# yhhshb/biolib

Hardware: AMD Instinct MI355X
Metric: Gbp/s minimizer-scanned (k=31,w=11) (higher is better)
Workload: dtype u64

## Files before the change

biolib_amd/csrc/bl_capi.hip:

```cpp
#include <hip/hip_runtime.h>
#include <algorithm>
#include <cstdio>
#include <cstdlib>
#include <cstring>
#include <deque>
#include <new>
#include <string>
#include <utility>
#include <vector>

#include "../../include/biolib_amd.h"
#include "bl_host.hpp"
#include "bl_launch.hpp"
#include "bl_lookup_launch.hpp"
#include "bl_read_counts_launch.hpp"
#include "bl_scan128_launch.hpp"

namespace {

thread_local std::string g_err;

int fail(int code, const std::string& msg)
{
    g_err = msg;
// ... 1 lines not shown
}

}

int bl_set_error(int code, const char* msg) { return fail(code, msg ? msg : ""); }

namespace {

#define BL_HIP(call)                                                                                       \
    do {                                                                                                   \
        hipError_t e_ = (call);                                                                            \
        if (e_ != hipSuccess)                                                                              \
            return fail(e_ == hipErrorOutOfMemory ? BL_ERR_OOM : BL_ERR_HIP,                               \
                        std::string(#call) + ": " + hipGetErrorString(e_));                                \
    } while (0)

constexpr int RESULT_WORDS = 16;
constexpr int RING = 256;
constexpr size_t HDR_BYTES = 256;
constexpr size_t SHARD_BYTES = (size_t)bl::NSHARD * 8 * sizeof(unsigned long long);

struct Pending {
    bl_result* user;
    int slot;
    uint64_t capacity;
    bool has_capacity;
};

}

struct Lane {
    hipStream_t own = nullptr;
    unsigned char* ws = nullptr;
    size_t ws_bytes = 0;
    unsigned char* tile_buf = nullptr;
    size_t tile_buf_bytes = 0;
    uint16_t* slot_buf = nullptr;
    size_t slot_buf_bytes = 0;
    hipEvent_t ev_start = nullptr, ev_stop = nullptr;
    hipEvent_t ev_count_done = nullptr;
    bool count_recorded = false;
    bool scan_recorded = false;

    unsigned long long* shards() const { return reinterpret_cast<unsigned long long*>(ws + HDR_BYTES); }
    unsigned long long* result() const { return reinterpret_cast<unsigned long long*>(ws + HDR_BYTES + SHARD_BYTES); }
};

struct bl_ctx {
    int device = 0;
    Lane lanes[2];
    Lane* cur = nullptr;
    int next_lane = 0;
    int n_lanes = 1;
    uint32_t emit_lds_per_wg = 0;
    hipStream_t user_stream = nullptr;
    bool borrowed = false;
    hipStream_t stream = nullptr;
    unsigned long long* pinned = nullptr;
    hipEvent_t slot_ev[RING] = {};
    int next_slot = 0;
    std::deque<Pending> pending;
    bool timed = false;
    bool exact_windows = false;
    bool position_tiled = false;
    bool packed_codes = true;
    bool direct_codes = true;
    int jaccard128_path = 0;
    bool count128_tables = true;
    int table_prefix_bits = -1;
    bool ktiming = false;
    bl::LaunchLog last_kernels{};
    std::vector<hipEvent_t> ev_pool;
    std::vector<std::pair<hipEvent_t, hipEvent_t>> ev_open;
    double kernel_ms = 0.0;
    uint64_t kernel_launches = 0;
    std::vector<std::pair<hipEvent_t, hipEvent_t>> marks;
    std::vector<bl_batch*> batches;
    void* scratch[8] = {};
    size_t scratch_bytes[8] = {};
    std::vector<std::pair<void*, size_t>> pool_idle;
    std::vector<std::pair<void*, size_t>> pool_live;

    unsigned long long* shards() const { return cur->shards(); }
    unsigned long long* result() const { return cur->result(); }
    static size_t fixed_bytes() { return HDR_BYTES + SHARD_BYTES + RESULT_WORDS * sizeof(unsigned long long); }
};

struct bl_batch {
    bl_ctx* ctx = nullptr;
    uint8_t* bases = nullptr;
    bool owns_bases = false;
    uint32_t* start_bits = nullptr;
    uint32_t* packed = nullptr;
    uint32_t* codes = nullptr;
    uint32_t* chunk_bad = nullptr;
    uint64_t n_bases = 0;
    uint64_t n_seqs = 0;
    uint64_t read_len = 0;
    uint64_t origin = 0;
};

namespace {

int grow(bl_ctx* c, void** buf, size_t* have, size_t need)
{
    if (need <= *have) return BL_OK;
    BL_HIP(hipStreamSynchronize(c->stream));
    if (*buf) BL_HIP(hipFree(*buf));
    *buf = nullptr;
    *have = 0;
    const size_t bytes = need + need / 8;
    hipError_t e = hipMalloc(buf, bytes);
    if (e != hipSuccess) return fail(BL_ERR_OOM, std::string("hipMalloc(scan scratch): ") + hipGetErrorString(e));
    *have = bytes;
    return BL_OK;
}

int ensure_workspace(bl_ctx* c)
{
    return grow(c, reinterpret_cast<void**>(&c->cur->ws), &c->cur->ws_bytes, bl_ctx::fixed_bytes());
}

void select_lane(bl_ctx* c)
{
    if (c->borrowed) {
        c->cur = &c->lanes[0];
        c->stream = c->user_stream;
    } else {
        c->cur = &c->lanes[c->next_lane];
        if (c->n_lanes == 2) c->next_lane ^= 1;
        c->stream = c->cur->own;
    }
}

void deliver(bl_ctx* c, const Pending& p)
{
    const unsigned long long* r = c->pinned + (size_t)p.slot * RESULT_WORDS;
    bl_result out;
    std::memset(&out, 0, sizeof(out));
    out.count = r[0];
    out.xor_value = r[1];
    out.xor_hash = r[2];
    out.xor_pos = r[3];
    out.aux = r[4];
    out.redone = (int32_t)(r[5] > 0x7fffffffull ? 0x7fffffffull : r[5]);
    out.status = BL_OK;
    if (p.has_capacity && r[0] > p.capacity) out.status = BL_ERR_CAPACITY;
    if (p.user) *p.user = out;
}

int flush_pending(bl_ctx* c)
{
// ... 18 lines not shown

int sync_ctx(bl_ctx* c)
{
    for (Lane& l : c->lanes) BL_HIP(hipStreamSynchronize(l.own));
    if (c->borrowed) BL_HIP(hipStreamSynchronize(c->user_stream));
    int rc = flush_kernel_events(c);
    if (rc != BL_OK) return rc;
    return flush_pending(c);
}

int kernel_event(bl_ctx* c, bool start)
{
    if (!c->ktiming) return BL_OK;
    if (start) {
        hipEvent_t ev[2];
        for (int i = 0; i < 2; ++i) {
            if (!c->ev_pool.empty()) { ev[i] = c->ev_pool.back(); c->ev_pool.pop_back(); }
            else BL_HIP(hipEventCreate(&ev[i]));
        }
        c->ev_open.emplace_back(ev[0], ev[1]);
        BL_HIP(hipEventRecord(ev[0], c->stream));
    } else {
        BL_HIP(hipEventRecord(c->ev_open.back().second, c->stream));
    }
    return BL_OK;
}

int begin_scan(bl_ctx* c)
{
    BL_HIP(hipSetDevice(c->device));
    select_lane(c);
    int rc = ensure_workspace(c);
    if (rc != BL_OK) return rc;
    BL_HIP(hipEventRecord(c->cur->ev_start, c->stream));
    BL_HIP(hipMemsetAsync(c->cur->ws, 0, bl_ctx::fixed_bytes(), c->stream));
    return BL_OK;
}

int end_scan(bl_ctx* c, uint32_t add_mask, bl_result* user, bool has_capacity, uint64_t capacity, uint32_t flags,
             bool already_folded = false)
{
    if (!already_folded) {
        hipError_t e = bl::launch_reduce_shards(c->shards(), c->result(), add_mask, reinterpret_cast<unsigned long long*>(c->cur->ws) + 1, c->stream);
        if (e != hipSuccess) return fail(BL_ERR_HIP, std::string("reduce_shards: ") + hipGetErrorString(e));
    }
    if ((int)c->pending.size() >= RING) {
        const Pending old = c->pending.front();
        BL_HIP(hipEventSynchronize(c->slot_ev[old.slot]));
        deliver(c, old);
        c->pending.pop_front();
    }
    const int slot = c->next_slot;
    c->next_slot = (c->next_slot + 1) % RING;
    BL_HIP(hipMemcpyAsync(c->pinned + (size_t)slot * RESULT_WORDS, c->result(), RESULT_WORDS * sizeof(unsigned long long),
                          hipMemcpyDeviceToHost, c->stream));
    BL_HIP(hipEventRecord(c->slot_ev[slot], c->stream));
    BL_HIP(hipEventRecord(c->cur->ev_stop, c->stream));
    c->cur->scan_recorded = true;
    c->timed = true;
    c->pending.push_back(Pending{user, slot, capacity, has_capacity});
    if (flags & BL_FLAG_SYNC) {
        int rc = sync_ctx(c);
        if (rc != BL_OK) return rc;
        if (user && user->status != BL_OK)
            return fail(user->status, "output capacity too small for the records found");
    }
    return BL_OK;
}

int zero_result(bl_ctx* c, bl_result* user, uint32_t flags)
{
    if (user) std::memset(user, 0, sizeof(*user));
    (void)c;
    (void)flags;
    return BL_OK;
}

int check_range(const bl_batch* b, uint64_t first, uint64_t n, uint64_t& end)
{
    if (first > b->n_bases) return fail(BL_ERR_INVALID, "range starts beyond the batch");
    end = (n == 0 || n > b->n_bases - first) ? b->n_bases : first + n;
    if (end - first > (1ull << 31)) return fail(BL_ERR_INVALID, "a scan range may hold at most 2^31 positions; split it");
    return BL_OK;
}

int make_start_bits(bl_ctx* c, bl_batch* b, const uint64_t* offsets, uint64_t n_seqs, uint64_t read_len)
{
    const uint64_t n_words = (b->n_bases + 31) / 32 + 4;
    if (!offsets && (read_len == 0 || read_len >= b->n_bases)) {
        b->start_bits = nullptr;
// ... 29 lines not shown
    const uint64_t total = (uint64_t)bl::packed_total((int64_t)b->n_bases);
    b->packed = static_cast<uint32_t*>(bl_ctx_pool_alloc(c, (total + total / 32) * sizeof(uint32_t)));
    if (!b->packed) return fail(BL_ERR_OOM, "device allocation of the batch's packed codes failed (bl_ctx_set_option(\"packed_codes\", 0) does without)");
    b->codes = b->packed + bl::PACK_LEAD;
    b->chunk_bad = b->packed + total + bl::PACK_LEAD / 32;
    hipError_t e = bl::launch_pack_codes(b->bases, b->n_bases, b->packed, b->packed + total, s);
    if (e != hipSuccess) return fail(BL_ERR_HIP, std::string("pack_codes: ") + hipGetErrorString(e));
    return BL_OK;
}

int ensure_start_bits(bl_ctx* c, const bl_batch* cb)
{
    bl_batch* b = const_cast<bl_batch*>(cb);
    if (b->start_bits || b->read_len == 0 || b->read_len >= b->n_bases) return BL_OK;
    int rc = sync_ctx(c);
    if (rc != BL_OK) return rc;
    return make_start_bits(c, b, nullptr, 0, b->read_len);
}

}

int bl_ctx_kernel_event(bl_ctx* c, hipStream_t stream, int start)
{
    const hipStream_t keep = c->stream;
    c->stream = stream;
    const int rc = kernel_event(c, start != 0);
    c->stream = keep;
    return rc;
}

hipStream_t bl_ctx_stream(bl_ctx* c)
{
    if (c->borrowed) return c->user_stream;
    if (c->n_lanes == 2 && c->lanes[1].scan_recorded) (void)hipStreamWaitEvent(c->lanes[0].own, c->lanes[1].ev_stop, 0);
    return c->lanes[0].own;
}
int bl_ctx_device(bl_ctx* c) { return c->device; }
int bl_ctx_count128_tables(bl_ctx* c) { return c->count128_tables ? 1 : 0; }
int bl_ctx_jaccard128_path(bl_ctx* c) { return c->jaccard128_path; }
int bl_ctx_table_prefix_bits(bl_ctx* c) { return c->table_prefix_bits; }
int bl_batch_describe(const bl_batch* b, bl_ctx** ctx, uint64_t* n_bases, uint64_t* n_seqs, uint64_t* read_len)
{
    *ctx = b->ctx;
    *n_bases = b->n_bases;
    *n_seqs = b->n_seqs;
    *read_len = b->read_len;
    return BL_OK;
}

int bl_batch_scan_view(bl_ctx* c, const bl_batch* b, int ensure, const uint32_t** start_bits)
{
    if (ensure) {
        int rc = ensure_start_bits(c, b);
        if (rc != BL_OK) return rc;
    }
    *start_bits = b->start_bits;
    return BL_OK;
}

void* bl_ctx_scratch(bl_ctx* c, int slot, size_t bytes)
{
    if (!c || slot < 0 || slot >= 8) return nullptr;
    if (bytes <= c->scratch_bytes[slot]) return c->scratch[slot];
    (void)hipSetDevice(c->device);
    if (c->scratch[slot]) {
        (void)hipDeviceSynchronize();
        (void)hipFree(c->scratch[slot]);
// ... 55 lines not shown
const char* bl_last_error(void) { return g_err.c_str(); }
int bl_version(void) { return BL_VERSION; }

int bl_device_count(int* n)
{
    if (!n) return fail(BL_ERR_INVALID, "n is NULL");
    int c = 0;
    hipError_t e = hipGetDeviceCount(&c);
    if (e != hipSuccess) { *n = 0; return fail(BL_ERR_NO_DEVICE, std::string("hipGetDeviceCount: ") + hipGetErrorString(e)); }
    *n = c;
    return BL_OK;
}

int bl_ctx_create(int device, bl_ctx** out)
{
    if (!out) return fail(BL_ERR_INVALID, "out is NULL");
    *out = nullptr;
    int n = 0;
    if (hipGetDeviceCount(&n) != hipSuccess || n == 0) return fail(BL_ERR_NO_DEVICE, "no HIP device visible: this library has no CPU fallback");
    if (device < 0 || device >= n) return fail(BL_ERR_INVALID, "device index out of range");
    hipDeviceProp_t prop;
    BL_HIP(hipGetDeviceProperties(&prop, device));
    if (std::strncmp(prop.gcnArchName, "gfx950", 6) != 0)
        return fail(BL_ERR_NO_DEVICE, std::string("device is ") + prop.gcnArchName + ", kernels are built for gfx950 (MI355X) only");
    BL_HIP(hipSetDevice(device));
    bl_ctx* c = new (std::nothrow) bl_ctx();
    if (!c) return fail(BL_ERR_OOM, "host allocation failed");
    c->device = device;
    hipError_t e = hipSuccess;
    for (Lane& l : c->lanes) {
        if (e == hipSuccess) e = hipStreamCreateWithFlags(&l.own, hipStreamNonBlocking);
        if (e == hipSuccess) e = hipEventCreate(&l.ev_start);
        if (e == hipSuccess) e = hipEventCreateWithFlags(&l.ev_count_done, hipEventDisableTiming);
        if (e == hipSuccess) e = hipEventCreate(&l.ev_stop);
    }
    if (e == hipSuccess) e = hipHostMalloc(reinterpret_cast<void**>(&c->pinned), (size_t)RING * RESULT_WORDS * sizeof(unsigned long long), hipHostMallocDefault);
    for (int i = 0; i < RING && e == hipSuccess; ++i) e = hipEventCreateWithFlags(&c->slot_ev[i], hipEventDisableTiming);
    if (e != hipSuccess) {
        bl_ctx_destroy(c);
        return fail(BL_ERR_HIP, std::string("context setup: ") + hipGetErrorString(e));
    }
    for (int i = 0; i < 2; ++i) {
        c->cur = &c->lanes[i];
        c->stream = c->cur->own;
        int rc = ensure_workspace(c);
        if (rc != BL_OK) { bl_ctx_destroy(c); return rc; }
    }
    c->cur = &c->lanes[0];
    c->stream = c->lanes[0].own;
    *out = c;
    return BL_OK;
}

int bl_ctx_set_lanes(bl_ctx* c, int n)
{
    if (!c || (n != 1 && n != 2)) return fail(BL_ERR_INVALID, "bl_ctx_set_lanes: need a context and n = 1 or 2");
    int rc = sync_ctx(c);
    if (rc != BL_OK) return rc;
    c->n_lanes = n;
    c->next_lane = 0;
    c->lanes[0].count_recorded = c->lanes[1].count_recorded = false;
    return BL_OK;
}

int bl_ctx_destroy(bl_ctx* c)
{
    if (!c) return BL_OK;
    (void)hipSetDevice(c->device);
    for (Lane& l : c->lanes)
        if (l.own) (void)hipStreamSynchronize(l.own);
    if (c->borrowed) (void)hipStreamSynchronize(c->user_stream);
    while (!c->batches.empty()) bl_batch_destroy(c->batches.back());
    for (Lane& l : c->lanes) {
        if (l.ws) (void)hipFree(l.ws);
        if (l.tile_buf) (void)hipFree(l.tile_buf);
        if (l.slot_buf) (void)hipFree(l.slot_buf);
        if (l.ev_start) (void)hipEventDestroy(l.ev_start);
        if (l.ev_count_done) (void)hipEventDestroy(l.ev_count_done);
        if (l.ev_stop) (void)hipEventDestroy(l.ev_stop);
        if (l.own) (void)hipStreamDestroy(l.own);
    }
    for (void* p : c->scratch)
        if (p) (void)hipFree(p);
    for (const auto& e : c->pool_idle) (void)hipFree(e.first);
    for (const auto& e : c->pool_live) (void)hipFree(e.first);
    if (c->pinned) (void)hipHostFree(c->pinned);
    for (hipEvent_t ev : c->slot_ev)
        if (ev) (void)hipEventDestroy(ev);
    for (auto& pr : c->ev_open) { (void)hipEventDestroy(pr.first); (void)hipEventDestroy(pr.second); }
    for (hipEvent_t ev : c->ev_pool) (void)hipEventDestroy(ev);
    for (auto& pr : c->marks) { (void)hipEventDestroy(pr.first); if (pr.second) (void)hipEventDestroy(pr.second); }
    delete c;
    return BL_OK;
}

int bl_ctx_set_stream(bl_ctx* c, void* hip_stream)
{
    if (!c) return fail(BL_ERR_INVALID, "ctx is NULL");
    int rc = sync_ctx(c);
    if (rc != BL_OK) return rc;
    c->borrowed = true;
    c->user_stream = static_cast<hipStream_t>(hip_stream);
    c->cur = &c->lanes[0];
    c->stream = c->user_stream;
    return BL_OK;
}

int bl_ctx_use_own_streams(bl_ctx* c)
{
    if (!c) return fail(BL_ERR_INVALID, "ctx is NULL");
    int rc = sync_ctx(c);
    if (rc != BL_OK) return rc;
    c->borrowed = false;
    c->user_stream = nullptr;
    c->cur = &c->lanes[0];
    c->stream = c->lanes[0].own;
    return BL_OK;
}

int bl_ctx_sync(bl_ctx* c)
{
    if (!c) return fail(BL_ERR_INVALID, "ctx is NULL");
    return sync_ctx(c);
}

int bl_ctx_last_scan_ms(bl_ctx* c, float* ms)
{
    if (!c || !ms) return fail(BL_ERR_INVALID, "NULL argument");
    if (!c->timed) return fail(BL_ERR_INVALID, "no scan has been issued on this context");
    BL_HIP(hipEventSynchronize(c->cur->ev_stop));
    BL_HIP(hipEventElapsedTime(ms, c->cur->ev_start, c->cur->ev_stop));
    return BL_OK;
}

int bl_ctx_set_exact_windows(bl_ctx* c, int on)
{
    if (!c) return fail(BL_ERR_INVALID, "ctx is NULL");
    c->exact_windows = on != 0;
    return BL_OK;
}

int bl_ctx_set_option(bl_ctx* c, const char* name, int64_t value)
{
    if (!c || !name) return fail(BL_ERR_INVALID, "bl_ctx_set_option: NULL argument");
    const std::string n(name);
    if (n == "exact_windows" && (value == 0 || value == 1)) return bl_ctx_set_exact_windows(c, (int)value);
    if (n == "lanes") return bl_ctx_set_lanes(c, (int)value);
    if (n == "position_tiled" && (value == 0 || value == 1)) {
        c->position_tiled = value != 0;
        return BL_OK;
    }
    if (n == "packed_codes" && (value == 0 || value == 1)) {
        c->packed_codes = value != 0;
        return BL_OK;
    }
    if (n == "direct_codes" && (value == 0 || value == 1)) {
        c->direct_codes = value != 0;
        return BL_OK;
    }
    if (n == "count128_tables" && (value == 0 || value == 1)) {
        c->count128_tables = value != 0;
        return BL_OK;
    }
    if (n == "jaccard128_path" && value >= 0 && value <= 2) {
// ... 368 lines not shown
static int scan_two_pass128(bl_ctx* c, P& p, bl::Kmer128Params& km, size_t lane_bytes, uint32_t** lane_rest, bool wants, uint64_t capacity, uint32_t flags,
                            bl_result* result, hipError_t (*count)(const P&, hipStream_t), hipError_t (*emit)(const P&, hipStream_t), const char* family)
{
    km.capacity = wants ? capacity : 0;
    int rc = begin_scan(c);
    if (rc != BL_OK) return rc;
    const size_t nt = (size_t)km.n_tiles, nb = (nt + bl::SCAN_BLK - 1) / bl::SCAN_BLK;
    rc = grow(c, reinterpret_cast<void**>(&c->cur->tile_buf), &c->cur->tile_buf_bytes, (2 * nt + 2 * nb + 8) * sizeof(unsigned long long));
    if (rc != BL_OK) return rc;
    unsigned long long* tb = reinterpret_cast<unsigned long long*>(c->cur->tile_buf);
    km.tile_counts = tb;
    km.tile_base = tb + nt;
    unsigned long long* block_tot = tb + 2 * nt;
    km.block_base = block_tot + nb;
    if (lane_bytes) {
        rc = grow(c, reinterpret_cast<void**>(&c->cur->slot_buf), &c->cur->slot_buf_bytes, nt * bl::TPB * lane_bytes);
        if (rc != BL_OK) return rc;
        km.lane_masks = c->cur->slot_buf;
        if (lane_rest) *lane_rest = reinterpret_cast<uint32_t*>(c->cur->slot_buf + nt * bl::TPB);
    }
    km.shards = c->shards();
    rc = kernel_event(c, true);
    if (rc != BL_OK) return rc;
    hipError_t e = count(p, c->stream);
    if (e != hipSuccess) return fail(BL_ERR_HIP, std::string(family) + "_count_kernel: " + hipGetErrorString(e));
    rc = kernel_event(c, false);
    if (rc != BL_OK) return rc;
    bl::ScanParams sp{};
    sp.tile_counts = km.tile_counts;
    sp.tile_base = km.tile_base;
    sp.block_base = km.block_base;
    sp.shards = km.shards;
    unsigned long long* carry = reinterpret_cast<unsigned long long*>(c->cur->ws);
    e = bl::launch_tile_scan(sp, bl::GroupRange{0, (uint32_t)km.n_tiles}, block_tot, carry, c->stream);
    if (e != hipSuccess) return fail(BL_ERR_HIP, std::string("tile_scan: ") + hipGetErrorString(e));
    if (wants) {
        e = emit(p, c->stream);
        if (e != hipSuccess) return fail(BL_ERR_HIP, std::string(family) + "_emit_kernel: " + hipGetErrorString(e));
    }
    return end_scan(c, 1u << 0, result, wants, capacity, flags);
}
}

int bl_scan_kmers128(bl_ctx* c, const bl_batch* b, uint64_t first, uint64_t n, uint32_t k, uint64_t seed, uint32_t flags,
                     uint64_t* d_values, uint64_t* d_hashes, uint8_t* d_valid, bl_result* result)
{
    bl::Kmer128Params p{};
    bool empty;
    int rc = prepare_kmers128(c, b, first, n, k, seed, flags, d_values, p, result, empty);
    if (rc != BL_OK || empty) return rc;
    p.out_value = d_values;
    p.out_hash = d_hashes;
    p.out_valid = d_valid;
    rc = begin_scan(c);
    if (rc != BL_OK) return rc;
    p.shards = c->shards();
    rc = kernel_event(c, true);
    if (rc != BL_OK) return rc;
    hipError_t e = bl::launch_kmers128(p, c->stream);
    if (e != hipSuccess) return fail(BL_ERR_HIP, std::string("kmer128_kernel: ") + hipGetErrorString(e));
    rc = kernel_event(c, false);
    if (rc != BL_OK) return rc;
    return end_scan(c,  (1u << 0) | (1u << 3), result, false, 0, flags);
}

int bl_scan_kmer_counts(bl_ctx* c, const bl_batch* b, uint64_t first, uint64_t n, uint32_t k, uint32_t flags, const bl_table* table, uint32_t* d_counts,
                        uint8_t* d_valid, bl_result* result)
// ... 160 lines not shown
    const size_t list_bytes = n_lists * slot_entries * sizeof(uint16_t);
    const size_t code_bytes = p.codes_packed ? 0 : nt * (size_t)p.slot_chunks * sizeof(uint32_t);
    rc = grow(c, reinterpret_cast<void**>(&c->cur->slot_buf), &c->cur->slot_buf_bytes, list_bytes + code_bytes);
    if (rc != BL_OK) return rc;
    unsigned long long* tb = reinterpret_cast<unsigned long long*>(c->cur->tile_buf);
    p.tile_counts = tb;
    p.tile_base = tb + nt;
    unsigned long long* block_tot = tb + 2 * nt;
    p.block_base = block_tot + nb;
    p.redo_list = reinterpret_cast<uint32_t*>(tb + 2 * nt + 2 * nb + 8);
    p.redo_count = reinterpret_cast<unsigned long long*>(c->cur->ws) + 1;
    p.slots_a = c->cur->slot_buf;
    p.slots_j = mode == bl::MODE_SUPERKMER ? c->cur->slot_buf + slot_entries : nullptr;
    p.slots_e = mode == bl::MODE_SUPERKMER ? c->cur->slot_buf + 2 * slot_entries : nullptr;
    p.slots_c = p.codes_packed ? nullptr : reinterpret_cast<uint32_t*>(reinterpret_cast<unsigned char*>(c->cur->slot_buf) + list_bytes);
    p.shards = c->shards();
    const bl::GroupRange all{0, (uint32_t)p.n_tiles};
    unsigned long long* carry = reinterpret_cast<unsigned long long*>(c->cur->ws);
    const bool staggered = c->n_lanes == 2 && !c->borrowed;
    if (staggered) {
        Lane* other = c->cur == &c->lanes[0] ? &c->lanes[1] : &c->lanes[0];
        if (other->count_recorded) BL_HIP(hipStreamWaitEvent(c->stream, other->ev_count_done, 0));
    }
    rc = kernel_event(c, true);
    if (rc != BL_OK) return rc;
    hipError_t e = bl::launch_scan_count(mode, p, all, c->stream, &c->last_kernels);
    if (e != hipSuccess) return fail(BL_ERR_HIP, std::string("scan_count_kernel: ") + hipGetErrorString(e));
    if (staggered) {
        BL_HIP(hipEventRecord(c->cur->ev_count_done, c->stream));
        c->cur->count_recorded = true;
    }
    rc = kernel_event(c, false);
    if (rc != BL_OK) return rc;
    e = bl::launch_tile_scan(p, all, block_tot, carry, c->stream);
    if (e != hipSuccess) return fail(BL_ERR_HIP, std::string("tile_scan: ") + hipGetErrorString(e));
    const uint32_t emit_lds_default = mode == bl::MODE_SUPERKMER ? 8192u : 28672u;
    e = bl::launch_scan_emit(mode, p, all, c->stream, staggered ? (c->emit_lds_per_wg ? c->emit_lds_per_wg : emit_lds_default) : 0, &c->last_kernels);
    if (e != hipSuccess) return fail(BL_ERR_HIP, std::string("scan_emit_kernel: ") + hipGetErrorString(e));
    return BL_OK;
}

int bl_scan_minimizers(bl_ctx* c, const bl_batch* b, uint64_t first, uint64_t n, uint32_t unit, uint32_t w, uint64_t seed, uint32_t flags,
                       uint64_t* d_values, uint64_t* d_positions, uint64_t* d_hashes, uint64_t capacity, bl_result* result)
{
    bl::ScanParams p{};
    p.out_value = d_values;
    p.out_pos = d_positions;
    p.out_hash = d_hashes;
    const bool wants = d_values || d_positions || d_hashes;
    int rc = scan_windows(bl::MODE_MINIMIZER, c, b, first, n, unit, w, seed, flags, p, wants ? capacity : 0, result);
    if (rc != BL_OK || p.n_tiles == 0) return rc;
    return end_scan(c, 1u << 0, result, wants, capacity, flags);
}

int bl_scan_hash_sample(bl_ctx* c, const bl_batch* b, uint64_t first, uint64_t n, uint32_t k, uint64_t seed, uint64_t threshold, uint32_t flags,
                        uint64_t* d_values, uint64_t* d_positions, uint64_t* d_hashes, uint64_t capacity, bl_result* result)
{
    bl::ScanParams p{};
    p.out_value = d_values;
    p.out_pos = d_positions;
    p.out_hash = d_hashes;
    p.use_threshold = 1;
    p.hash_below = threshold;
    const bool wants = d_values || d_positions || d_hashes;
    int rc = scan_windows(bl::MODE_MINIMIZER, c, b, first, n, k, 1, seed, flags, p, wants ? capacity : 0, result);
    if (rc != BL_OK || p.n_tiles == 0) return rc;
    return end_scan(c, 1u << 0, result, wants, capacity, flags);
// ... 159 lines not shown
```

biolib_amd/csrc/bl_kernels.hip:

```cpp
#include <hip/hip_runtime.h>
#include <cstdlib>
#include "bl_scan_frl.hpp"
#include "bl_launch.hpp"

#ifndef BL_SY0_WAVES
#define BL_SY0_WAVES 2
#endif
#ifndef BL_SY2_WAVES
#define BL_SY2_WAVES 3
#endif
#ifndef BL_CS_WAVES
#define BL_CS_WAVES 3
#endif
#ifndef BL_POSAX_WAVES
#define BL_POSAX_WAVES 4
#endif
#ifndef BL_SKAX_WAVES
#define BL_SKAX_WAVES 4
#endif
#ifndef BL_C4_WAVES
#define BL_C4_WAVES 5
#endif
#ifndef BL_CSRT_WAVES
#define BL_CSRT_WAVES 3
// ... 379 lines not shown
    if constexpr (K > 1) {
        __shared__ uint32_t acc[6][TPB];
#pragma unroll
        for (int i = 0; i < 6; ++i) acc[i][tid] = 0;
        const uint32_t t0 = blockIdx.x * K;
#pragma unroll 1
        for (uint32_t k = 0; k < (uint32_t)K && t0 + k < g.count; ++k) {
            Digest d1{0, 0, 0};
            emit_tile<MODE, true, C3, false, PACKED>(p, codes[k & 1], g.first + t0 + k, tid, d1);
            acc[0][tid] ^= (uint32_t)d1.xv; acc[1][tid] ^= (uint32_t)(d1.xv >> 32);
            acc[2][tid] ^= (uint32_t)d1.xh; acc[3][tid] ^= (uint32_t)(d1.xh >> 32);
            acc[4][tid] ^= (uint32_t)d1.xp; acc[5][tid] ^= (uint32_t)(d1.xp >> 32);
        }
        dg.xv = ((unsigned long long)acc[1][tid] << 32) | acc[0][tid];
        dg.xh = ((unsigned long long)acc[3][tid] << 32) | acc[2][tid];
        dg.xp = ((unsigned long long)acc[5][tid] << 32) | acc[4][tid];
    } else {
        if (blockIdx.x >= g.count) return;
        emit_tile<MODE, false, C3, WIDE, PACKED>(p, codes[0], g.first + blockIdx.x, tid, dg);
    }

    const unsigned long long xv = MODE == MODE_SYNCMER ? 0ull : wave_xor_to_last_u64(dg.xv), xh = MODE == MODE_SYNCMER ? 0ull : wave_xor_to_last_u64(dg.xh);
    const unsigned long long xp = wave_xor_to_last_u64(dg.xp);
    if ((tid & 63) == 63 && (xv | xh | xp)) {
        unsigned long long* shard = p.shards + 8 * ((blockIdx.x * NWAVE + (tid >> 6)) % NSHARD);
        if (MODE != MODE_SYNCMER) {
            atomicXor(&shard[1], xv);
            atomicXor(&shard[2], xh);
        }
        atomicXor(&shard[3], xp);
    }
}

__global__ __launch_bounds__(512) void tile_scan_local_kernel(const unsigned long long* counts, unsigned long long* tile_base,
                                                              unsigned long long* block_tot, uint32_t first_tile, uint32_t n_group)
{
    __shared__ unsigned long long wtot[8];
    const int tid = threadIdx.x, lane = tid & 63, wv = tid >> 6;
    const uint32_t rel = blockIdx.x * SCAN_BLK + tid * 4;
    unsigned long long c[4], run = 0;
#pragma unroll
    for (int i = 0; i < 4; ++i) {
        c[i] = rel + i < n_group ? counts[first_tile + rel + i] : 0;
        run += c[i];
    }
    unsigned long long incl = run;
#pragma unroll
    for (int d = 1; d < 64; d <<= 1) {
        const unsigned long long o = __shfl_up(incl, d, 64);
        if (lane >= d) incl += o;
    }
    if (lane == 63) wtot[wv] = incl;
    __syncthreads();
    unsigned long long before = 0, all = 0;
#pragma unroll
    for (int i = 0; i < 8; ++i) {
        if (i < wv) before += wtot[i];
        all += wtot[i];
    }
    unsigned long long ex = before + incl - run;
#pragma unroll
    for (int i = 0; i < 4; ++i) {
        if (rel + i < n_group) tile_base[first_tile + rel + i] = ex;
        ex += c[i];
    }
    if (tid == 0) block_tot[first_tile / SCAN_BLK + blockIdx.x] = all;
}

__global__ void tile_scan_top_kernel(const unsigned long long* block_tot, unsigned long long* block_base, uint32_t first_block,
                                     uint32_t n_blocks, unsigned long long* carry, unsigned long long* shards)
{
    if (blockIdx.x != 0 || threadIdx.x >= 64) return;
    const uint32_t lane = threadIdx.x, per = (n_blocks + 63) / 64;
    const uint32_t lo = lane * per, hi = lo + per < n_blocks ? lo + per : n_blocks;
    unsigned long long sum = 0;
    for (uint32_t i = lo; i < hi; ++i) sum += block_tot[first_block + i];
    unsigned long long incl = sum;
#pragma unroll
    for (int d = 1; d < 64; d <<= 1) {
        const unsigned long long o = __shfl_up(incl, d, 64);
        if ((int)lane >= d) incl += o;
    }
    const unsigned long long before = *carry;
    unsigned long long run = before + incl - sum;
    for (uint32_t i = lo; i < hi; ++i) {
        block_base[first_block + i] = run;
        run += block_tot[first_block + i];
    }
    const unsigned long long total = __shfl(incl, 63, 64);
    if (lane == 0) {
        *carry = before + total;
        shards[0] += total & 0xffffffffull;
        shards[4] += total >> 32;
    }
}

struct KmerShared {
    uint32_t codes[NCHUNK_POS];
    uint32_t flags[NCHUNK_POS];
    unsigned long long dig[4];
};

__global__ __launch_bounds__(TPB) void kmer_kernel(const KmerParams p)
{
    __shared__ KmerShared sh;
    const int tid = threadIdx.x;
    KmerAcc acc{0, 0, 0, 0};
    if (tid < 4) sh.dig[tid] = 0;
    ScanParams lp{};
    lp.bases = p.bases;
    lp.n_bases = p.n_bases;
    lp.start_bits = p.start_bits;
    for (int tile = blockIdx.x; tile < p.n_tiles; tile += gridDim.x) {
        const int64_t q0 = p.origin + (int64_t)tile * H;
        __syncthreads();
        stage_chunk(lp, sh.codes, sh.flags, tid, q0);
        if (tid < NCHUNK_POS - TPB) stage_chunk(lp, sh.codes, sh.flags, TPB + tid, q0);
        __syncthreads();
        kmer_thread(p, sh.codes, sh.flags, tid, q0, acc);
    }
    __syncthreads();
    const unsigned long long c = wave_sum_u64(acc.cnt), xv = wave_xor_u64(acc.xv), xh = wave_xor_u64(acc.xh), s = wave_sum_u64(acc.sh);
    if ((tid & 63) == 0) {
        atomicAdd(&sh.dig[0], c);
        atomicXor(&sh.dig[1], xv);
        atomicXor(&sh.dig[2], xh);
        atomicAdd(&sh.dig[3], s);
    }
    __syncthreads();
    if (tid < 4) {
        unsigned long long* shard = p.shards + 8 * (blockIdx.x % NSHARD);
        if (tid == 0 || tid == 3) atomicAdd(&shard[tid], sh.dig[tid]);
        else atomicXor(&shard[tid], sh.dig[tid]);
    }
}


__global__ void reduce_shards_kernel(const unsigned long long* shards, unsigned long long* result, uint32_t add_mask, const unsigned long long* redone)
{
    const int slot = threadIdx.x;
    if (slot == 8) result[8] = 0;
    if (slot == 9) result[5] = *redone;
    if (slot >= 8) return;
    if (slot == 5) return;
    unsigned long long acc = 0;
    for (int i = 0; i < NSHARD; ++i) {
        const unsigned long long v = shards[8 * i + slot];
        if ((add_mask >> slot) & 1) acc += v;
        else acc ^= v;
    }
    result[slot] = acc;
}

__global__ void synth_kernel(uint8_t* bases, uint64_t first, uint64_t n, uint64_t seed)
{
    const uint64_t wordi = (uint64_t)blockIdx.x * blockDim.x + threadIdx.x;
    const uint64_t i0 = wordi * 32;
    if (i0 >= n) return;
    uint64_t x = seed + ((first + i0) >> 5);
    x += 0x9E3779B97F4A7C15ULL;
    x = (x ^ (x >> 30)) * 0xBF58476D1CE4E5B9ULL;
    x = (x ^ (x >> 27)) * 0x94D049BB133111EBULL;
    x ^= x >> 31;
    const uint32_t lut = 0x54474341u;
    uint32_t out[8];
#pragma unroll
    for (int q = 0; q < 8; ++q) {
        const uint32_t c4 = (uint32_t)(x >> (8 * q)) & 0xffu;
        const uint32_t sel = (c4 & 3u) | (((c4 >> 2) & 3u) << 8) | (((c4 >> 4) & 3u) << 16) | (((c4 >> 6) & 3u) << 24);
        out[q] = __builtin_amdgcn_perm(lut, lut, sel);
    }
    if (i0 + 32 <= n) {
        uint4* dst = reinterpret_cast<uint4*>(bases + i0);
        dst[0] = make_uint4(out[0], out[1], out[2], out[3]);
        dst[1] = make_uint4(out[4], out[5], out[6], out[7]);
    } else {
        for (uint64_t b = 0; i0 + b < n; ++b) bases[i0 + b] = (uint8_t)(out[b >> 2] >> (8 * (b & 3)));
    }
}

__global__ void start_bits_fixed_kernel(uint32_t* bits, uint64_t n_words, uint64_t n_bases, uint64_t read_len)
{
    const uint64_t wi = (uint64_t)blockIdx.x * blockDim.x + threadIdx.x;
    if (wi >= n_words) return;
// ... 211 lines not shown
    const dim3 grid((g.count + K - 1) / K), block(TPB);
    if (MODE == MODE_MINIMIZER && p.frl && p.unit == 31 && p.canonical) {
        const uint32_t have_c3 = (uint32_t)(((K > 1 ? 2 : 1) * 2 * C3_RC + (K > 1 ? 6 * TPB : 0)) * sizeof(uint32_t));
        if (p.codes_packed) BL_LAUNCH("emit<MM,C3>", (scan_emit_kernel<MODE_MINIMIZER, 31, 1, 1, false, true>), grid, block, lds_per_wg > have_c3 ? lds_per_wg - have_c3 : 0, p, g);
        else BL_LAUNCH("emit<MM,C3>", (scan_emit_kernel<MODE_MINIMIZER, 31, 1, 1>), grid, block, lds_per_wg > have_c3 ? lds_per_wg - have_c3 : 0, p, g);
        return;
    }
    if (MODE == MODE_SUPERKMER && p.records128) {
        if (p.codes_packed) BL_LAUNCH("emit<SK,wide>", (scan_emit_kernel<MODE_SUPERKMER, 0, -1, -1, true, true>), grid, block, pad, p, g);
        else BL_LAUNCH("emit<SK,wide>", (scan_emit_kernel<MODE_SUPERKMER, 0, -1, -1, true>), grid, block, pad, p, g);
        return;
    }
    if (MODE != MODE_SYNCMER && p.codes_packed) BL_LAUNCH(BL_MODE_NAME("emit<", ">"), (scan_emit_kernel<MODE, 0, -1, -1, false, MODE != MODE_SYNCMER>), grid, block, pad, p, g);
    else BL_LAUNCH(BL_MODE_NAME("emit<", ">"), (scan_emit_kernel<MODE>), grid, block, pad, p, g);
}

hipError_t launch_scan_emit(int mode, const ScanParams& p, GroupRange g, hipStream_t stream, uint32_t lds_per_wg, LaunchLog* log)
{
    if (g.count == 0) return hipSuccess;
    switch (mode) {
        case MODE_MINIMIZER: launch_emit_mode<MODE_MINIMIZER>(p, g, stream, lds_per_wg, log); break;
        case MODE_SUPERKMER: launch_emit_mode<MODE_SUPERKMER>(p, g, stream, lds_per_wg, log); break;
        case MODE_SYNCMER: launch_emit_mode<MODE_SYNCMER>(p, g, stream, lds_per_wg, log); break;
        default: return hipErrorInvalidValue;
    }
    return hipGetLastError();
}
#undef BL_LAUNCH
#undef BL_PK
#undef BL_PK_W
#undef BL_MODE_NAME
#undef BL_W_ALL

hipError_t launch_tile_scan(const ScanParams& p, GroupRange g, unsigned long long* block_tot, unsigned long long* carry, hipStream_t stream)
{
    if (g.count == 0) return hipSuccess;
    const uint32_t n_blocks = (g.count + SCAN_BLK - 1) / SCAN_BLK;
    hipLaunchKernelGGL(tile_scan_local_kernel, dim3(n_blocks), dim3(512), 0, stream, p.tile_counts, p.tile_base, block_tot, g.first, g.count);
    hipLaunchKernelGGL(tile_scan_top_kernel, dim3(1), dim3(64), 0, stream, block_tot, p.block_base, g.first / SCAN_BLK, n_blocks, carry,
                       p.shards);
    return hipGetLastError();
}

hipError_t launch_kmers(const KmerParams& p, int n_blocks, hipStream_t stream)
{
    if (p.n_tiles <= 0) return hipSuccess;
    hipLaunchKernelGGL(kmer_kernel, dim3(n_blocks), dim3(TPB), 0, stream, p);
    return hipGetLastError();
}

hipError_t launch_reduce_shards(const unsigned long long* shards, unsigned long long* result, uint32_t add_mask, const unsigned long long* redone, hipStream_t stream)
{
    hipLaunchKernelGGL(reduce_shards_kernel, dim3(1), dim3(64), 0, stream, shards, result, add_mask, redone);
    return hipGetLastError();
}

hipError_t launch_synth(uint8_t* bases, uint64_t first, uint64_t n, uint64_t seed, hipStream_t stream)
{
    if (n == 0) return hipSuccess;
    const uint64_t words = (n + 31) / 32;
    hipLaunchKernelGGL(synth_kernel, dim3((unsigned)((words + 255) / 256)), dim3(256), 0, stream, bases, first, n, seed);
    return hipGetLastError();
}

hipError_t launch_start_bits_fixed(uint32_t* bits, uint64_t n_words, uint64_t n_bases, uint64_t read_len, hipStream_t stream)
{
    if (n_words == 0) return hipSuccess;
    hipLaunchKernelGGL(start_bits_fixed_kernel, dim3((unsigned)((n_words + 255) / 256)), dim3(256), 0, stream, bits, n_words, n_bases, read_len);
    return hipGetLastError();
}

hipError_t launch_start_bits_offsets(uint32_t* bits, const uint64_t* offsets, uint64_t n_seqs, uint64_t n_bases, hipStream_t stream)
{
    if (n_seqs == 0) return hipSuccess;
    hipLaunchKernelGGL(start_bits_offsets_kernel, dim3((unsigned)((n_seqs + 255) / 256)), dim3(256), 0, stream, bits, offsets, n_seqs, n_bases);
    return hipGetLastError();
}

hipError_t launch_pack_codes(const uint8_t* bases, uint64_t n_bases, uint32_t* codes, uint32_t* chunk_bad, hipStream_t stream)
{
    const uint64_t total = (uint64_t)packed_total((int64_t)n_bases);
    hipLaunchKernelGGL(pack_codes_kernel, dim3((unsigned)((total + 255) / 256)), dim3(256), 0, stream, bases, (int64_t)n_bases, codes, chunk_bad);
    return hipGetLastError();
}

}
// ... 11 lines not shown
```

biolib_amd/csrc/bl_launch.hpp:

```cpp
#pragma once
#include <hip/hip_runtime.h>
#include "bl_scan_phases.hpp"

namespace bl {
struct LaunchLog {
    static constexpr int MAX = 8;
    const char* names[MAX];
    int n;
    void add(const char* name) { if (n < MAX) names[n++] = name; }
};
const char* const* scan_kernel_names(int* count);
hipError_t launch_scan_count(int mode, const ScanParams& p, GroupRange g, hipStream_t stream, LaunchLog* log);
hipError_t launch_scan_emit(int mode, const ScanParams& p, GroupRange g, hipStream_t stream, uint32_t lds_per_wg, LaunchLog* log);
hipError_t launch_tile_scan(const ScanParams& p, GroupRange g, unsigned long long* block_tot, unsigned long long* carry, hipStream_t stream);
hipError_t launch_kmers(const KmerParams& p, int n_blocks, hipStream_t stream);
hipError_t launch_reduce_shards(const unsigned long long* shards, unsigned long long* result, uint32_t add_mask, const unsigned long long* redone, hipStream_t stream);
hipError_t launch_synth(uint8_t* bases, uint64_t first, uint64_t n, uint64_t seed, hipStream_t stream);
hipError_t launch_start_bits_fixed(uint32_t* bits, uint64_t n_words, uint64_t n_bases, uint64_t read_len, hipStream_t stream);
hipError_t launch_start_bits_offsets(uint32_t* bits, const uint64_t* offsets, uint64_t n_seqs, uint64_t n_bases, hipStream_t stream);
hipError_t launch_pack_codes(const uint8_t* bases, uint64_t n_bases, uint32_t* codes, uint32_t* chunk_bad, hipStream_t stream);
}
```

Before: 604.1.

## Fuse tile-scan passes and fold shard reduction, readback and rezeroing into one kernel

```diff
diff --git a/biolib_amd/csrc/bl_capi.hip b/biolib_amd/csrc/bl_capi.hip
--- a/biolib_amd/csrc/bl_capi.hip
+++ b/biolib_amd/csrc/bl_capi.hip
@@ -57,18 +57,19 @@
 struct Lane {
     hipStream_t own = nullptr;
     unsigned char* ws = nullptr;
+    bool ws_zero = false;
     size_t ws_bytes = 0;
     unsigned char* tile_buf = nullptr;
     size_t tile_buf_bytes = 0;
     uint16_t* slot_buf = nullptr;
     size_t slot_buf_bytes = 0;
-    hipEvent_t ev_start = nullptr, ev_stop = nullptr;
+    hipEvent_t ev_start = nullptr;
+    hipEvent_t stop = nullptr;
     hipEvent_t ev_count_done = nullptr;
     bool count_recorded = false;
     bool scan_recorded = false;
 
     unsigned long long* shards() const { return reinterpret_cast<unsigned long long*>(ws + HDR_BYTES); }
-    unsigned long long* result() const { return reinterpret_cast<unsigned long long*>(ws + HDR_BYTES + SHARD_BYTES); }
 };
 
 struct bl_ctx {
@@ -107,8 +108,7 @@
     std::vector<std::pair<void*, size_t>> pool_live;
 
     unsigned long long* shards() const { return cur->shards(); }
-    unsigned long long* result() const { return cur->result(); }
-    static size_t fixed_bytes() { return HDR_BYTES + SHARD_BYTES + RESULT_WORDS * sizeof(unsigned long long); }
+    static size_t fixed_bytes() { return HDR_BYTES + SHARD_BYTES; }
 };
 
 struct bl_batch {
@@ -143,6 +143,7 @@
 
 int ensure_workspace(bl_ctx* c)
 {
+    if (bl_ctx::fixed_bytes() > c->cur->ws_bytes) c->cur->ws_zero = false;
     return grow(c, reinterpret_cast<void**>(&c->cur->ws), &c->cur->ws_bytes, bl_ctx::fixed_bytes());
 }
 
@@ -227,18 +228,15 @@
     select_lane(c);
     int rc = ensure_workspace(c);
     if (rc != BL_OK) return rc;
+    const bool zero = c->cur->ws_zero;
+    c->cur->ws_zero = false;
     BL_HIP(hipEventRecord(c->cur->ev_start, c->stream));
-    BL_HIP(hipMemsetAsync(c->cur->ws, 0, bl_ctx::fixed_bytes(), c->stream));
-    return BL_OK;
-}
-
-int end_scan(bl_ctx* c, uint32_t add_mask, bl_result* user, bool has_capacity, uint64_t capacity, uint32_t flags,
-             bool already_folded = false)
-{
-    if (!already_folded) {
-        hipError_t e = bl::launch_reduce_shards(c->shards(), c->result(), add_mask, reinterpret_cast<unsigned long long*>(c->cur->ws) + 1, c->stream);
-        if (e != hipSuccess) return fail(BL_ERR_HIP, std::string("reduce_shards: ") + hipGetErrorString(e));
-    }
+    if (!zero) BL_HIP(hipMemsetAsync(c->cur->ws, 0, bl_ctx::fixed_bytes(), c->stream));
+    return BL_OK;
+}
+
+int end_scan(bl_ctx* c, uint32_t add_mask, bl_result* user, bool has_capacity, uint64_t capacity, uint32_t flags)
+{
     if ((int)c->pending.size() >= RING) {
         const Pending old = c->pending.front();
         BL_HIP(hipEventSynchronize(c->slot_ev[old.slot]));
@@ -247,10 +245,13 @@
     }
     const int slot = c->next_slot;
     c->next_slot = (c->next_slot + 1) % RING;
-    BL_HIP(hipMemcpyAsync(c->pinned + (size_t)slot * RESULT_WORDS, c->result(), RESULT_WORDS * sizeof(unsigned long long),
-                          hipMemcpyDeviceToHost, c->stream));
+    unsigned long long* hdr = reinterpret_cast<unsigned long long*>(c->cur->ws);
+    hipError_t e = bl::launch_scan_finish(hdr, (uint32_t)(HDR_BYTES / sizeof(unsigned long long)), c->shards(), c->pinned + (size_t)slot * RESULT_WORDS,
+                                          RESULT_WORDS, add_mask, hdr + 1, c->stream);
+    if (e != hipSuccess) return fail(BL_ERR_HIP, std::string("scan_finish: ") + hipGetErrorString(e));
+    c->cur->ws_zero = true;
     BL_HIP(hipEventRecord(c->slot_ev[slot], c->stream));
-    BL_HIP(hipEventRecord(c->cur->ev_stop, c->stream));
+    c->cur->stop = c->slot_ev[slot];
     c->cur->scan_recorded = true;
     c->timed = true;
     c->pending.push_back(Pending{user, slot, capacity, has_capacity});
@@ -346,7 +347,7 @@
 hipStream_t bl_ctx_stream(bl_ctx* c)
 {
     if (c->borrowed) return c->user_stream;
-    if (c->n_lanes == 2 && c->lanes[1].scan_recorded) (void)hipStreamWaitEvent(c->lanes[0].own, c->lanes[1].ev_stop, 0);
+    if (c->n_lanes == 2 && c->lanes[1].scan_recorded) (void)hipStreamWaitEvent(c->lanes[0].own, c->lanes[1].stop, 0);
     return c->lanes[0].own;
 }
 int bl_ctx_device(bl_ctx* c) { return c->device; }
@@ -468,10 +469,9 @@
         if (e == hipSuccess) e = hipStreamCreateWithFlags(&l.own, hipStreamNonBlocking);
         if (e == hipSuccess) e = hipEventCreate(&l.ev_start);
         if (e == hipSuccess) e = hipEventCreateWithFlags(&l.ev_count_done, hipEventDisableTiming);
-        if (e == hipSuccess) e = hipEventCreate(&l.ev_stop);
     }
     if (e == hipSuccess) e = hipHostMalloc(reinterpret_cast<void**>(&c->pinned), (size_t)RING * RESULT_WORDS * sizeof(unsigned long long), hipHostMallocDefault);
-    for (int i = 0; i < RING && e == hipSuccess; ++i) e = hipEventCreateWithFlags(&c->slot_ev[i], hipEventDisableTiming);
+    for (int i = 0; i < RING && e == hipSuccess; ++i) e = hipEventCreate(&c->slot_ev[i]);
     if (e != hipSuccess) {
         bl_ctx_destroy(c);
         return fail(BL_ERR_HIP, std::string("context setup: ") + hipGetErrorString(e));
@@ -496,6 +496,7 @@
     c->n_lanes = n;
     c->next_lane = 0;
     c->lanes[0].count_recorded = c->lanes[1].count_recorded = false;
+    c->lanes[0].ws_zero = c->lanes[1].ws_zero = false;
     return BL_OK;
 }
 
@@ -513,7 +514,6 @@
         if (l.slot_buf) (void)hipFree(l.slot_buf);
         if (l.ev_start) (void)hipEventDestroy(l.ev_start);
         if (l.ev_count_done) (void)hipEventDestroy(l.ev_count_done);
-        if (l.ev_stop) (void)hipEventDestroy(l.ev_stop);
         if (l.own) (void)hipStreamDestroy(l.own);
     }
     for (void* p : c->scratch)
@@ -563,9 +563,9 @@
 int bl_ctx_last_scan_ms(bl_ctx* c, float* ms)
 {
     if (!c || !ms) return fail(BL_ERR_INVALID, "NULL argument");
-    if (!c->timed) return fail(BL_ERR_INVALID, "no scan has been issued on this context");
-    BL_HIP(hipEventSynchronize(c->cur->ev_stop));
-    BL_HIP(hipEventElapsedTime(ms, c->cur->ev_start, c->cur->ev_stop));
+    if (!c->timed || !c->cur->stop) return fail(BL_ERR_INVALID, "no scan has been issued on this context");
+    BL_HIP(hipEventSynchronize(c->cur->stop));
+    BL_HIP(hipEventElapsedTime(ms, c->cur->ev_start, c->cur->stop));
     return BL_OK;
 }
 
@@ -1000,7 +1000,7 @@
     sp.block_base = km.block_base;
     sp.shards = km.shards;
     unsigned long long* carry = reinterpret_cast<unsigned long long*>(c->cur->ws);
-    e = bl::launch_tile_scan(sp, bl::GroupRange{0, (uint32_t)km.n_tiles}, block_tot, carry, c->stream);
+    e = bl::launch_tile_scan(sp, bl::GroupRange{0, (uint32_t)km.n_tiles}, block_tot, carry, reinterpret_cast<unsigned int*>(carry + 2), c->stream);
     if (e != hipSuccess) return fail(BL_ERR_HIP, std::string("tile_scan: ") + hipGetErrorString(e));
     if (wants) {
         e = emit(p, c->stream);
@@ -1227,7 +1227,7 @@
     }
     rc = kernel_event(c, false);
     if (rc != BL_OK) return rc;
-    e = bl::launch_tile_scan(p, all, block_tot, carry, c->stream);
+    e = bl::launch_tile_scan(p, all, block_tot, carry, reinterpret_cast<unsigned int*>(carry + 2), c->stream);
     if (e != hipSuccess) return fail(BL_ERR_HIP, std::string("tile_scan: ") + hipGetErrorString(e));
     const uint32_t emit_lds_default = mode == bl::MODE_SUPERKMER ? 8192u : 28672u;
     e = bl::launch_scan_emit(mode, p, all, c->stream, staggered ? (c->emit_lds_per_wg ? c->emit_lds_per_wg : emit_lds_default) : 0, &c->last_kernels);
diff --git a/biolib_amd/csrc/bl_kernels.hip b/biolib_amd/csrc/bl_kernels.hip
--- a/biolib_amd/csrc/bl_kernels.hip
+++ b/biolib_amd/csrc/bl_kernels.hip
@@ -435,8 +435,9 @@
     }
 }
 
-__global__ __launch_bounds__(512) void tile_scan_local_kernel(const unsigned long long* counts, unsigned long long* tile_base,
-                                                              unsigned long long* block_tot, uint32_t first_tile, uint32_t n_group)
+__global__ __launch_bounds__(512) void tile_scan_kernel(const unsigned long long* counts, unsigned long long* tile_base,
+                                                        unsigned long long* block_tot, unsigned long long* block_base, uint32_t first_tile,
+                                                        uint32_t n_group, unsigned long long* carry, unsigned long long* shards, unsigned int* ticket)
 {
     __shared__ unsigned long long wtot[8];
     const int tid = threadIdx.x, lane = tid & 63, wv = tid >> 6;
@@ -467,34 +468,37 @@
         if (rel + i < n_group) tile_base[first_tile + rel + i] = ex;
         ex += c[i];
     }
-    if (tid == 0) block_tot[first_tile / SCAN_BLK + blockIdx.x] = all;
-}
-
-__global__ void tile_scan_top_kernel(const unsigned long long* block_tot, unsigned long long* block_base, uint32_t first_block,
-                                     uint32_t n_blocks, unsigned long long* carry, unsigned long long* shards)
-{
-    if (blockIdx.x != 0 || threadIdx.x >= 64) return;
-    const uint32_t lane = threadIdx.x, per = (n_blocks + 63) / 64;
-    const uint32_t lo = lane * per, hi = lo + per < n_blocks ? lo + per : n_blocks;
+    if (wv != 0) return;
+    const uint32_t first_block = first_tile / SCAN_BLK, n_blocks = gridDim.x;
+    unsigned int drawn = 0;
+    if (tid == 0) {
+        __hip_atomic_store(&block_tot[first_block + blockIdx.x], all, __ATOMIC_RELAXED, __HIP_MEMORY_SCOPE_AGENT);
+        asm volatile("s_waitcnt vmcnt(0)" ::: "memory");
+        drawn = __hip_atomic_fetch_add(ticket, 1u, __ATOMIC_RELAXED, __HIP_MEMORY_SCOPE_AGENT);
+    }
+    if ((unsigned int)__builtin_amdgcn_readfirstlane((int)drawn) != n_blocks - 1) return;
+    const uint32_t per = (n_blocks + 63) / 64;
+    const uint32_t lo = (uint32_t)lane * per, hi = lo + per < n_blocks ? lo + per : n_blocks;
     unsigned long long sum = 0;
-    for (uint32_t i = lo; i < hi; ++i) sum += block_tot[first_block + i];
-    unsigned long long incl = sum;
+    for (uint32_t i = lo; i < hi; ++i) sum += __hip_atomic_load(&block_tot[first_block + i], __ATOMIC_RELAXED, __HIP_MEMORY_SCOPE_AGENT);
+    unsigned long long tincl = sum;
 #pragma unroll
     for (int d = 1; d < 64; d <<= 1) {
-        const unsigned long long o = __shfl_up(incl, d, 64);
-        if ((int)lane >= d) incl += o;
-    }
-    const unsigned long long before = *carry;
-    unsigned long long run = before + incl - sum;
+        const unsigned long long o = __shfl_up(tincl, d, 64);
+        if (lane >= d) tincl += o;
+    }
+    const unsigned long long prev = *carry;
+    unsigned long long trun = prev + tincl - sum;
     for (uint32_t i = lo; i < hi; ++i) {
-        block_base[first_block + i] = run;
-        run += block_tot[first_block + i];
-    }
-    const unsigned long long total = __shfl(incl, 63, 64);
+        block_base[first_block + i] = trun;
+        trun += __hip_atomic_load(&block_tot[first_block + i], __ATOMIC_RELAXED, __HIP_MEMORY_SCOPE_AGENT);
+    }
+    const unsigned long long total = __shfl(tincl, 63, 64);
     if (lane == 0) {
-        *carry = before + total;
+        *carry = prev + total;
         shards[0] += total & 0xffffffffull;
         shards[4] += total >> 32;
+        __hip_atomic_store(ticket, 0u, __ATOMIC_RELAXED, __HIP_MEMORY_SCOPE_AGENT);
     }
 }
 
@@ -539,20 +543,35 @@
 }
 
 
-__global__ void reduce_shards_kernel(const unsigned long long* shards, unsigned long long* result, uint32_t add_mask, const unsigned long long* redone)
-{
-    const int slot = threadIdx.x;
-    if (slot == 8) result[8] = 0;
-    if (slot == 9) result[5] = *redone;
-    if (slot >= 8) return;
-    if (slot == 5) return;
-    unsigned long long acc = 0;
-    for (int i = 0; i < NSHARD; ++i) {
-        const unsigned long long v = shards[8 * i + slot];
-        if ((add_mask >> slot) & 1) acc += v;
-        else acc ^= v;
-    }
-    result[slot] = acc;
+__global__ __launch_bounds__(NSHARD) void scan_finish_kernel(unsigned long long* hdr, uint32_t hdr_words, unsigned long long* shards,
+                                                             unsigned long long* record, uint32_t record_words, uint32_t add_mask,
+                                                             const unsigned long long* redone)
+{
+    static_assert(NSHARD == 256, "one thread per shard, four waves");
+    __shared__ unsigned long long part[NSHARD / 64][8];
+    const int tid = threadIdx.x;
+    const unsigned long long redo = *redone;
+    unsigned long long v[8];
+#pragma unroll
+    for (int s = 0; s < 8; ++s) v[s] = shards[8 * tid + s];
+#pragma unroll
+    for (int s = 0; s < 8; ++s) {
+        v[s] = ((add_mask >> s) & 1u) ? wave_sum_u64(v[s]) : wave_xor_u64(v[s]);
+        if ((tid & 63) == 0) part[tid >> 6][s] = v[s];
+    }
+    __syncthreads();
+    if (tid < (int)record_words) {
+        unsigned long long r = 0;
+        if (tid == 5) r = redo;
+        else if (tid < 8) {
+#pragma unroll
+            for (int wv = 0; wv < NSHARD / 64; ++wv) r = ((add_mask >> tid) & 1u) ? r + part[wv][tid] : r ^ part[wv][tid];
+        }
+        record[tid] = r;
+    }
+#pragma unroll
+    for (int s = 0; s < 8; ++s) shards[8 * tid + s] = 0;
+    if (tid < (int)hdr_words) hdr[tid] = 0;
 }
 
 __global__ void synth_kernel(uint8_t* bases, uint64_t first, uint64_t n, uint64_t seed)
@@ -830,13 +849,13 @@
 #undef BL_MODE_NAME
 #undef BL_W_ALL
 
-hipError_t launch_tile_scan(const ScanParams& p, GroupRange g, unsigned long long* block_tot, unsigned long long* carry, hipStream_t stream)
+hipError_t launch_tile_scan(const ScanParams& p, GroupRange g, unsigned long long* block_tot, unsigned long long* carry, unsigned int* ticket,
+                            hipStream_t stream)
 {
     if (g.count == 0) return hipSuccess;
     const uint32_t n_blocks = (g.count + SCAN_BLK - 1) / SCAN_BLK;
-    hipLaunchKernelGGL(tile_scan_local_kernel, dim3(n_blocks), dim3(512), 0, stream, p.tile_counts, p.tile_base, block_tot, g.first, g.count);
-    hipLaunchKernelGGL(tile_scan_top_kernel, dim3(1), dim3(64), 0, stream, block_tot, p.block_base, g.first / SCAN_BLK, n_blocks, carry,
-                       p.shards);
+    hipLaunchKernelGGL(tile_scan_kernel, dim3(n_blocks), dim3(512), 0, stream, p.tile_counts, p.tile_base, block_tot, p.block_base, g.first, g.count,
+                       carry, p.shards, ticket);
     return hipGetLastError();
 }
 
@@ -847,9 +866,11 @@
     return hipGetLastError();
 }
 
-hipError_t launch_reduce_shards(const unsigned long long* shards, unsigned long long* result, uint32_t add_mask, const unsigned long long* redone, hipStream_t stream)
-{
-    hipLaunchKernelGGL(reduce_shards_kernel, dim3(1), dim3(64), 0, stream, shards, result, add_mask, redone);
+hipError_t launch_scan_finish(unsigned long long* hdr, uint32_t hdr_words, unsigned long long* shards, unsigned long long* record,
+                              uint32_t record_words, uint32_t add_mask, const unsigned long long* redone, hipStream_t stream)
+{
+    if (hdr_words > (uint32_t)NSHARD || record_words > (uint32_t)NSHARD) return hipErrorInvalidValue;
+    hipLaunchKernelGGL(scan_finish_kernel, dim3(1), dim3(NSHARD), 0, stream, hdr, hdr_words, shards, record, record_words, add_mask, redone);
     return hipGetLastError();
 }
 
diff --git a/biolib_amd/csrc/bl_launch.hpp b/biolib_amd/csrc/bl_launch.hpp
--- a/biolib_amd/csrc/bl_launch.hpp
+++ b/biolib_amd/csrc/bl_launch.hpp
@@ -12,9 +12,11 @@
 const char* const* scan_kernel_names(int* count);
 hipError_t launch_scan_count(int mode, const ScanParams& p, GroupRange g, hipStream_t stream, LaunchLog* log);
 hipError_t launch_scan_emit(int mode, const ScanParams& p, GroupRange g, hipStream_t stream, uint32_t lds_per_wg, LaunchLog* log);
-hipError_t launch_tile_scan(const ScanParams& p, GroupRange g, unsigned long long* block_tot, unsigned long long* carry, hipStream_t stream);
+hipError_t launch_tile_scan(const ScanParams& p, GroupRange g, unsigned long long* block_tot, unsigned long long* carry, unsigned int* ticket,
+                            hipStream_t stream);
 hipError_t launch_kmers(const KmerParams& p, int n_blocks, hipStream_t stream);
-hipError_t launch_reduce_shards(const unsigned long long* shards, unsigned long long* result, uint32_t add_mask, const unsigned long long* redone, hipStream_t stream);
+hipError_t launch_scan_finish(unsigned long long* hdr, uint32_t hdr_words, unsigned long long* shards, unsigned long long* record,
+                              uint32_t record_words, uint32_t add_mask, const unsigned long long* redone, hipStream_t stream);
 hipError_t launch_synth(uint8_t* bases, uint64_t first, uint64_t n, uint64_t seed, hipStream_t stream);
 hipError_t launch_start_bits_fixed(uint32_t* bits, uint64_t n_words, uint64_t n_bases, uint64_t read_len, hipStream_t stream);
 hipError_t launch_start_bits_offsets(uint32_t* bits, const uint64_t* offsets, uint64_t n_seqs, uint64_t n_bases, hipStream_t stream);
```

Result: no change. 603.0, median of 3 (-0.2%).
